# mfkiwl/GPS-JAMMING

Measured on AMD Instinct MI355X. Metric: Msamples/s uint8 I/Q through PSD+TDOA xcorr, higher is better.
Workload: dtype f32

## Files before the change

### gps-jamming_amd/csrc/k_scan.hip

```cpp
#include <type_traits>

#include "gj_common.h"

namespace gj {

constexpr int kScanThreads = 256;
constexpr size_t kScanTile = 65536;

__device__ __forceinline__ void acc_moments(const uint4& q, unsigned& s2, unsigned& s1) {
    s2 = __builtin_amdgcn_udot4(q.x, q.x, s2, false);
    s2 = __builtin_amdgcn_udot4(q.y, q.y, s2, false);
    s2 = __builtin_amdgcn_udot4(q.z, q.z, s2, false);
    s2 = __builtin_amdgcn_udot4(q.w, q.w, s2, false);
    s1 = __builtin_amdgcn_udot4(q.x, 0x01010101u, s1, false);
    s1 = __builtin_amdgcn_udot4(q.y, 0x01010101u, s1, false);
    s1 = __builtin_amdgcn_udot4(q.z, 0x01010101u, s1, false);
    s1 = __builtin_amdgcn_udot4(q.w, 0x01010101u, s1, false);
}

__device__ __forceinline__ void block_byte_moments(const uint8_t* __restrict__ p, size_t begin, size_t end,
                                                   unsigned long long& s2_out, unsigned long long& s1_out) {
    __shared__ unsigned long long red[2][kScanThreads / 64];
    const int tid = threadIdx.x;
    unsigned s2 = 0, s1 = 0;
// ... 163 lines not shown
                    run_len = 0;
                }
                ++run_len;
            }
        });
        if (run_len) atomicAdd(&sh.hist[run_digit], run_len);
        __syncthreads();
        const unsigned h = sh.hist[tid];
        unsigned inc = h;
#pragma unroll
        for (int off = 1; off < 64; off <<= 1) {
            const unsigned o = __shfl_up(inc, off, 64);
            if ((tid & 63) >= off) inc += o;
        }
        if ((tid & 63) == 63) sh.wave_tot[tid >> 6] = inc;
        __syncthreads();
        unsigned base = 0;
        for (int w = 0; w < (tid >> 6); ++w) base += sh.wave_tot[w];
        const unsigned excl = base + inc - h;
        if (h && excl <= want && want < excl + h) { sh.digit = tid; sh.rest = want - excl; }
        __syncthreads();
        prefix |= sh.digit << shift;
        mask |= 255u << shift;
        want = sh.rest;
        __syncthreads();
    }
    return prefix;
}

__device__ __forceinline__ void power_threshold_body(const float* __restrict__ power, size_t n, float pct, float ratio,
                                                     float* __restrict__ stats, uint8_t* __restrict__ mask, ThrShared& sh) {
    const int tid = threadIdx.x;
    const bool cached = n <= (size_t)kThrCache;
    if (tid == 0) { sh.nan_flag = 0; sh.above = 0; sh.count_le = 0; sh.next_key = 0xffffffffu; }
    __syncthreads();
    unsigned reg[kThrPerThread];
    unsigned has_nan = 0;
    if (cached) {
#pragma unroll
        for (int j = 0; j < kThrPerThread; ++j) {
            const size_t i = (size_t)tid + (size_t)kThrThreads * j;
            const float p = (i < n) ? power[i] : 0.0f;
            has_nan |= (p != p);
            reg[j] = float_key(p);
        }
    } else {
#pragma unroll
        for (int j = 0; j < kThrPerThread; ++j) reg[j] = 0;
        for (size_t i = tid; i < n; i += kThrThreads) {
            const float p = power[i];
            has_nan |= (p != p);
        }
    }
    if (has_nan) atomicOr(&sh.nan_flag, 1u);
    const float q = pct / 100.0f;
    const float vidx = (float)(n - 1) * q;
    size_t lo = (size_t)floorf(vidx);
    if (lo > n - 1) lo = n - 1;
    const size_t hi = (lo + 1 < n) ? lo + 1 : n - 1;
    const float g = vidx - (float)lo;
    const unsigned ka = block_select(reg, power, cached, n, lo, sh);
    unsigned kb = ka;
    if (hi != lo) {
        unsigned cnt = 0, nxt = 0xffffffffu;
        thr_for_each(reg, power, cached, n, [&](unsigned k, size_t) {
            cnt += (k <= ka);
            if (k > ka && k < nxt) nxt = k;
        });
        cnt = wave_sum_u32(cnt);
#pragma unroll
        for (int off = 32; off > 0; off >>= 1) {
            const unsigned o = __shfl_xor(nxt, off, 64);
            nxt = o < nxt ? o : nxt;
        }
        if ((tid & 63) == 0) { atomicAdd(&sh.count_le, cnt); atomicMin(&sh.next_key, nxt); }
        __syncthreads();
        kb = (sh.count_le >= lo + 2) ? ka : sh.next_key;
    }
    if (tid == 0) {
        const float a = key_float(ka), b = key_float(kb);
        const float d = b - a;
        float base = (g >= 0.5f) ? (b - d * (1.0f - g)) : (a + d * g);
        if (sh.nan_flag) base = __builtin_nanf("");
        if (base <= 0.0f) base = 1.0f;
        const float thr = base * ratio;
        stats[0] = base;
        stats[1] = thr;
        sh.thr = thr;
    }
    __syncthreads();
    const float thr = sh.thr;
    unsigned cnt = 0;
    thr_for_each(reg, power, cached, n, [&](unsigned k, size_t i) {
        const bool hot = key_float(k) > thr;
        cnt += hot;
        if (mask) mask[i] = hot;
    });
    cnt = wave_sum_u32(cnt);
    if ((tid & 63) == 0) atomicAdd(&sh.above, (unsigned long long)cnt);
    __syncthreads();
    if (tid == 0) stats[2] = (float)sh.above;
}

__global__ __launch_bounds__(kThrThreads) __attribute__((amdgpu_num_vgpr(104))) void power_threshold_kernel(const float* __restrict__ power, size_t n, float pct,
                                                                      float ratio, float* __restrict__ stats,
                                                                      uint8_t* __restrict__ mask) {
    __shared__ ThrShared sh;
    power_threshold_body(power, n, pct, ratio, stats, mask, sh);
}

int launch_power_threshold(gj_ctx* ctx, const float* d_power, size_t n, float pct, float rise_db, float* d_stats,
                           uint8_t* d_mask) {
    if (n == 0) return fail(ctx, GJ_ERR_INVALID, "empty power map");
    const float ratio = (float)pow(10.0, (double)rise_db / 10.0);
    hipLaunchKernelGGL(power_threshold_kernel, dim3(1), dim3(kThrThreads), 0, ctx->stream, d_power, n, pct, ratio, d_stats,
                       d_mask);
    GJ_LAUNCH_CHECK(ctx);
    return GJ_OK;
}

__device__ __forceinline__ float amp_of(unsigned i8, unsigned q8, Unpack up) {
    const int vi = 2 * (int)i8 - up.off2, vq = 2 * (int)q8 - up.off2;
    return __fsqrt_rn((float)(vi * vi + vq * vq)) * up.half_scale;
}
__device__ __forceinline__ unsigned pk_minus_off2(int o2) { return ((unsigned)(-o2) & 0xffffu) * 0x10001u; }

template <int HI>
__device__ __forceinline__ float amp_of_half(unsigned w, unsigned k2, unsigned km255, float hs) {
    const unsigned spread = __builtin_amdgcn_perm(w, w, HI ? 0x0C030C02u : 0x0C010C00u);
    unsigned h;
    int m;
    asm("v_pk_mad_i16 %0, %1, %2, %3" : "=v"(h) : "v"(spread), "v"(k2), "v"(km255));
    asm("v_dot2_i32_i16 %0, %1, %1, 0" : "=v"(m) : "v"(h));
    return __fsqrt_rn((float)m) * hs;
}

__device__ __forceinline__ unsigned m_of(unsigned i8, unsigned q8, int o2 = 255) {
    const int vi = 2 * (int)i8 - o2, vq = 2 * (int)q8 - o2;
    return (unsigned)(vi * vi + vq * vq);
}

template <int HI>
__device__ __forceinline__ int msq_of_half(unsigned w, unsigned k2, unsigned km255) {
    const unsigned spread = __builtin_amdgcn_perm(w, w, HI ? 0x0C030C02u : 0x0C010C00u);
    unsigned h;
    int m;
    asm("v_pk_mad_i16 %0, %1, %2, %3" : "=v"(h) : "v"(spread), "v"(k2), "v"(km255));
    asm("v_dot2_i32_i16 %0, %1, %1, 0" : "=v"(m) : "v"(h));
    return m;
}

constexpr size_t kAmpTileSamples = kScanTile / 2;

struct AmpTile {
    double sum;
    long long first;
};

__device__ double block_sum_f64(double v, double* sh ) {
    v = wave_sum_f64(v);
    __syncthreads();
    if ((threadIdx.x & 63) == 0) sh[threadIdx.x >> 6] = v;
    __syncthreads();
    double t = 0.0;
    for (unsigned k = 0; k < blockDim.x / 64; ++k) t += sh[k];
    return t;
}

__device__ long long amp_block_first(const AmpTile* __restrict__ tiles, size_t ntiles, long long* first_s) {
    if (threadIdx.x == 0) *first_s = 0x7fffffffffffffffll;
    __syncthreads();
    long long f = 0x7fffffffffffffffll;
    for (size_t t = threadIdx.x; t < ntiles; t += 16 * (size_t)blockDim.x) {
        long long v[16];
#pragma unroll
        for (int k = 0; k < 16; ++k) {
            const size_t tt = t + (size_t)k * blockDim.x;
            v[k] = tt < ntiles ? tiles[tt].first : 0x7fffffffffffffffll;
        }
#pragma unroll
        for (int k = 0; k < 16; ++k) f = v[k] < f ? v[k] : f;
    }
    if (f != 0x7fffffffffffffffll) atomicMin(first_s, f);
    __syncthreads();
    return *first_s;
}

__device__ double amp_block_tail(const uint8_t* __restrict__ iq, size_t nsamples, const AmpTile* __restrict__ tiles,
                                 long long first, Unpack up, double* sh) {
    const size_t t0 = (size_t)first / kAmpTileSamples;
    if ((size_t)first == t0 * kAmpTileSamples) return tiles[t0].sum;
    const size_t e0 = ((t0 + 1) * kAmpTileSamples < nsamples) ? (t0 + 1) * kAmpTileSamples : nsamples;
    double acc = 0.0;
    for (size_t s = (size_t)first + threadIdx.x; s < e0; s += blockDim.x) acc += (double)amp_of(iq[2 * s], iq[2 * s + 1], up);
    return block_sum_f64(acc, sh);
}

__device__ double amp_block_total(const AmpTile* __restrict__ tiles, size_t ntiles, size_t t0, double* sh) {
    double acc = 0.0;
    for (size_t t = t0 + 1 + threadIdx.x; t < ntiles; t += 16 * (size_t)blockDim.x) {
        double v[16];
#pragma unroll
        for (int k = 0; k < 16; ++k) {
            const size_t tt = t + (size_t)k * blockDim.x;
            v[k] = tt < ntiles ? tiles[tt].sum : 0.0;
        }
#pragma unroll
        for (int g = 0; g < 2; ++g) {
            if (t + (size_t)(8 * g) * blockDim.x < ntiles)
                acc += ((v[8 * g] + v[8 * g + 1]) + (v[8 * g + 2] + v[8 * g + 3])) + ((v[8 * g + 4] + v[8 * g + 5]) + (v[8 * g + 6] + v[8 * g + 7]));
        }
    }
    return block_sum_f64(acc, sh);
}

static inline bool power_edge_value(size_t nchunks, size_t nbytes, size_t chunk_bytes, int flags, float* val) {
    if (!nchunks) return false;
    const size_t len = nbytes - (nchunks - 1) * chunk_bytes;
    if ((flags & GJ_CP_ODD_CHUNK_ZERO) && (len & 1)) { *val = 0.0f; return true; }
    if ((len >> 1) == 0) { *val = __builtin_nanf(""); return true; }
    return false;
}
__device__ __forceinline__ void amp_combine_body(const AmpTile* __restrict__ tiles, size_t ntiles,
                                                 const gj_amp_part* __restrict__ parts, int n_parts, size_t nsamples,
                                                 gj_amp_stats* __restrict__ out, double* sh) {
    long long first = 0x7fffffffffffffffll;
    double tail = 0.0;
    for (int p = 0; p < n_parts; ++p)
        if (parts[p].first_index >= 0 && parts[p].first_index < first) { first = parts[p].first_index; tail = parts[p].tail; }
    if (first == 0x7fffffffffffffffll) {
        if (threadIdx.x == 0) {
            out->first_index = -1; out->count = 0; out->sum = 0.0; out->mean = 0.f; out->reserved = 0.f;
        }
        return;
    }
    const double behind = amp_block_total(tiles, ntiles, (size_t)first / kAmpTileSamples, sh);
    if (threadIdx.x == 0) {
        const double total = behind + tail;
        const unsigned long long cnt = nsamples - (size_t)first;
        out->first_index = first;
        out->count = cnt;
        out->sum = total;
        out->mean = (float)(total / (double)cnt);
        out->reserved = 0.f;
    }
}

__global__ __launch_bounds__(256) void amp_combine_kernel(const AmpTile* __restrict__ tiles, size_t ntiles,
                                                           const gj_amp_part* __restrict__ parts, int n_parts,
                                                           size_t nsamples, gj_amp_stats* __restrict__ out) {
    __shared__ double sh[16];
    amp_combine_body(tiles, ntiles, parts, n_parts, nsamples, out, sh);
}

__global__ __launch_bounds__(kThrThreads) __attribute__((amdgpu_num_vgpr(104))) void combine_stats_kernel(
    const gj_combine_capture* __restrict__ caps, int n_captures, float pct, float ratio) {
    __shared__ ThrShared sh_thr;
    __shared__ double sh_amp[16];
    const int b = blockIdx.x;
    if (b < n_captures) {
        const gj_combine_capture c = caps[b];
        power_threshold_body(c.d_power, (size_t)c.n_chunks, pct, ratio, c.d_stats, nullptr, sh_thr);
    } else {
        const gj_combine_capture c = caps[b - n_captures];
        amp_combine_body(static_cast<const AmpTile*>(c.d_tiles), (size_t)c.n_tiles, c.d_amp_parts, c.n_parts,
                         (size_t)(c.total_bytes / 2), c.d_amp, sh_amp);
        if (threadIdx.x == 0) onset_combine(c.d_onset_parts, c.n_parts, c.d_onset);
    }
}

int launch_combine_stats(gj_ctx* ctx, const gj_combine_capture* d_caps, int n_captures, float pct, float rise_db) {
    const float ratio = (float)pow(10.0, (double)rise_db / 10.0);
    hipLaunchKernelGGL(combine_stats_kernel, dim3(2u * (unsigned)n_captures), dim3(kThrThreads), 0, ctx->stream, d_caps,
                       n_captures, pct, ratio);
    GJ_LAUNCH_CHECK(ctx);
    return GJ_OK;
}

constexpr int kOnsetOut = 2048;
constexpr int kOnsetMaxWin = 8192;

struct OnsetScratch {
    unsigned long long noise_S;
    float noise;
    float thr;
};

constexpr double kOnsetGuard = 1e-6;

__device__ __forceinline__ int onset_pad(int k) { return k + (k >> 5); }

typedef short gj_short2 __attribute__((ext_vector_type(2)));

__device__ __forceinline__ int wave_sum_lane63(int v) {
    v += __builtin_amdgcn_update_dpp(0, v, 0xB1, 0xf, 0xf, false);
    v += __builtin_amdgcn_update_dpp(0, v, 0x4E, 0xf, 0xf, false);
    v += __builtin_amdgcn_update_dpp(0, v, 0x141, 0xf, 0xf, false);
    v += __builtin_amdgcn_update_dpp(0, v, 0x140, 0xf, 0xf, false);
    v += __builtin_amdgcn_update_dpp(0, v, 0x142, 0xa, 0xf, false);
    v += __builtin_amdgcn_update_dpp(0, v, 0x143, 0xc, 0xf, false);
    return v;
}


template <bool TRACK_FIRST>
__global__ __launch_bounds__(kScanThreads) void stream_scan_kernel(const uint8_t* __restrict__ iq, size_t nsamples,
                                                                   size_t nbytes, size_t chunk_bytes,
                                                                   unsigned tiles_per_chunk, float eps, int flags,
                                                                   float* __restrict__ power,
                                                                   unsigned long long* __restrict__ acc, float thr,
                                                                   AmpTile* __restrict__ tiles,
                                                                   unsigned* __restrict__ cblk, Unpack up,
                                                                   unsigned skip_tiles, unsigned tile_base,
                                                                   unsigned noise_block, const uint8_t* __restrict__ noise_src,
                                                                   int noise_samples, OnsetScratch* __restrict__ sc) {
    if (blockIdx.x == noise_block) {
        unsigned long long s2 = 0, s1 = 0;
        block_byte_moments(noise_src, 0, (size_t)2 * noise_samples, s2, s1);
        if (threadIdx.x == 0)
            sc->noise_S = (unsigned long long)(4ll * (long long)s2 - 4ll * up.off2 * (long long)s1 + (long long)up.off2 * up.off2 * (2ll * noise_samples));
        return;
    }
    __shared__ unsigned long long red_m[2][kScanThreads / 64];
    __shared__ double red_s[kScanThreads / 64];
    __shared__ long long red_f[kScanThreads / 64];
    const int tid = threadIdx.x;
    const size_t t = (size_t)blockIdx.x + tile_base;
    const size_t b0 = t * kScanTile;
    const size_t use_end = 2 * nsamples;
    const size_t b1 = (b0 + kScanTile < use_end) ? b0 + kScanTile : use_end;
    const size_t nvec = (b1 - b0) >> 4;
    const uint4* v = reinterpret_cast<const uint4*>(iq + b0);
    unsigned S = 0;
    double sum = 0.0;
    long long first = 0x7fffffffffffffffll;
    unsigned k2 = 0x00020002u, km255 = pk_minus_off2(up.off2);
    asm volatile("" : "+v"(k2), "+v"(km255));
    auto body = [&](const uint4& q, unsigned i, const bool live) {
        const unsigned ws[4] = {q.x, q.y, q.z, q.w};
        int m[8];
#pragma unroll
        for (int k = 0; k < 4; ++k) {
            m[2 * k] = msq_of_half<0>(ws[k], k2, km255);
            m[2 * k + 1] = msq_of_half<1>(ws[k], k2, km255);
        }
        float part = 0.f;
#pragma unroll
        for (int k = 0; k < 8; ++k) {
            const float r = __fsqrt_rn((float)m[k]);
            part += r;
            if constexpr (TRACK_FIRST) {
                const long long idx = (long long)((b0 >> 1) + (size_t)i * 8 + k);
                if (live && r * up.half_scale > thr && idx < first) first = idx;
            }
        }
        const unsigned m8 = live ? (unsigned)(((m[0] + m[1]) + (m[2] + m[3])) + ((m[4] + m[5]) + (m[6] + m[7]))) : 0u;
        S += m8;
        const int c512 = wave_sum_lane63((int)m8);
        if ((tid & 63) == 63) cblk[(b0 >> 10) + (i >> 6)] = (unsigned)c512;
        sum += (double)(live ? part : 0.f);
    };
    if (nvec == kScanTile / 16) {
        for (unsigned i = tid; i < (unsigned)(kScanTile / 16); i += 4 * kScanThreads) {
            const uint4 q0 = v[i], q1 = v[i + kScanThreads], q2 = v[i + 2 * kScanThreads], q3 = v[i + 3 * kScanThreads];
            body(q0, i, true);
            body(q1, i + kScanThreads, true);
            body(q2, i + 2 * kScanThreads, true);
            body(q3, i + 3 * kScanThreads, true);
        }
    } else {
        const unsigned lane = tid & 63;
        for (unsigned ib = (unsigned)tid - lane; ib < (unsigned)nvec; ib += kScanThreads) {
            const unsigned i = ib + lane;
            const bool live = i < (unsigned)nvec;
            const uint4 q = live ? v[i] : uint4{0u, 0u, 0u, 0u};
            body(q, i, live);
        }
    }
    if (tid == 0 && (b0 + (nvec << 4)) < b1) {
        unsigned c = 0;
        for (size_t n = (b0 >> 1) + nvec * 8; 2 * n < b1; ++n) {
            const unsigned ui = iq[2 * n], uq = iq[2 * n + 1];
            const unsigned mm = m_of(ui, uq, up.off2);
            S += mm;
            c += mm;
            const float r = __fsqrt_rn((float)mm);
            sum += (double)r;
            if (TRACK_FIRST && r * up.half_scale > thr && (long long)n < first) first = (long long)n;
        }
        (void)c;
    }
    if (b1 == use_end && (b1 & 1023) != 0) {
        __syncthreads();
        if (tid < 64) {
            const size_t jb = (b1 - 1) >> 10;
            int c = 0;
            for (size_t n = jb * 512 + tid; n < nsamples; n += 64) c += (int)m_of(iq[2 * n], iq[2 * n + 1], up.off2);
            c = group_sum_dpp<64>(c);
            if (tid == 0) cblk[jb] = (unsigned)c;
        }
    }
    if constexpr (!TRACK_FIRST) {
        if (tid == 0 && b1 > b0) first = (long long)(b0 >> 1);
    }
    const unsigned long long mS = wave_sum_u64(S);
    sum = wave_sum_f64(sum);
#pragma unroll
    for (int off = 32; off > 0; off >>= 1) {
        const long long o = __shfl_xor(first, off, 64);
        first = o < first ? o : first;
    }
    if ((tid & 63) == 0) { red_m[0][tid >> 6] = mS; red_s[tid >> 6] = sum; red_f[tid >> 6] = first; }
    __syncthreads();
    if (tid == 0 && t >= skip_tiles) {
        const unsigned long long tS = red_m[0][0] + red_m[0][1] + red_m[0][2] + red_m[0][3];
        AmpTile at;
        at.sum = ((red_s[0] + red_s[1]) + (red_s[2] + red_s[3])) * (double)up.half_scale;
        long long f = red_f[0];
        for (int k = 1; k < 4; ++k) f = red_f[k] < f ? red_f[k] : f;
        at.first = (f == 0x7fffffffffffffffll) ? f : f - (long long)((size_t)skip_tiles * (kScanTile / 2));
        const size_t to = t - skip_tiles;
        tiles[to] = at;
        const size_t c = to / tiles_per_chunk;
        const size_t off = c * chunk_bytes;
        const size_t len = (nbytes - off < chunk_bytes) ? nbytes - off : chunk_bytes;
        const bool zero_rule = (flags & GJ_CP_ODD_CHUNK_ZERO) && ((len & 1) || len == 0);
        if (tiles_per_chunk == 1) {
            power[c] = zero_rule ? 0.0f : ((len >> 1) ? power_from_msum(tS, len >> 1, eps) : __builtin_nanf(""));
        } else {
            atomicAdd(&acc[2 * c], tS);
        }
    }
}

constexpr size_t kTailSlotBytes = 256u << 10;
constexpr size_t kTailPrioBytes = 256u << 20;
constexpr int kTailBlocks = 2048;
constexpr int kTailHalo = (kOnsetMaxWin + 510) / 512 + 1;
constexpr int kTailPre = kTailBlocks + kTailHalo + (kTailBlocks + kTailHalo) / 32 + 8;

struct TailRec {
    unsigned long long first;
    unsigned long long guard;
    unsigned below;
    unsigned pad;
};

struct TailArgs {
    const uint8_t* iq;
    unsigned long long nsamples;
    long long sample0;
    unsigned long long total_samples;
    unsigned long long slot_nsamples;
    int has_thr, is_part, valid, has_slot, hi_prio;
    float* power;
    unsigned long long nchunks;
    float pct, ratio;
    float* stats;
    uint8_t* mask;
    const uint8_t* own_iq;
    unsigned long long own_samples, own_tiles;
    const AmpTile* tiles;
    gj_amp_stats* amp;
    gj_amp_part* amp_part;
    long long own_sample0;
    int window, noise_samples, noise_in_scratch;
    float factor;
    const unsigned* cblk;
    OnsetScratch* sc;
    TailRec* rec;
    unsigned* arrive;
    unsigned nct;
    gj_onset* onset;
    uint8_t* slot;
    unsigned long long slice_samples;
    Unpack up;
};

struct TailShared {
    unsigned long long r64[2][kScanThreads / 64];
    unsigned r32[kScanThreads / 64];
    unsigned long long b64[2];
    unsigned b32;
    int last;
    long long start;
};

__device__ __forceinline__ unsigned long long block_min_u64(unsigned long long v, TailShared& sh, int slot) {
#pragma unroll
    for (int off = 32; off > 0; off >>= 1) {
        const unsigned long long o = __shfl_xor(v, off, 64);
        v = o < v ? o : v;
    }
    if ((threadIdx.x & 63) == 0) sh.r64[slot][threadIdx.x >> 6] = v;
    __syncthreads();
    unsigned long long r = sh.r64[slot][0];
#pragma unroll
    for (int k = 1; k < kScanThreads / 64; ++k) r = sh.r64[slot][k] < r ? sh.r64[slot][k] : r;
    __syncthreads();
    return r;
}
__device__ __forceinline__ unsigned block_max_u32(unsigned v, TailShared& sh) {
#pragma unroll
    for (int off = 32; off > 0; off >>= 1) {
        const unsigned o = __shfl_xor(v, off, 64);
        v = o > v ? o : v;
    }
    if ((threadIdx.x & 63) == 0) sh.r32[threadIdx.x >> 6] = v;
    __syncthreads();
    unsigned r = sh.r32[0];
#pragma unroll
    for (int k = 1; k < kScanThreads / 64; ++k) r = sh.r32[k] > r ? sh.r32[k] : r;
    __syncthreads();
    return r;
}
__device__ __forceinline__ unsigned long long block_sum_u64(unsigned long long v, TailShared& sh) {
    v = wave_sum_u64(v);
    if ((threadIdx.x & 63) == 0) sh.r64[0][threadIdx.x >> 6] = v;
    __syncthreads();
    unsigned long long r = 0;
#pragma unroll
    for (int k = 0; k < kScanThreads / 64; ++k) r += sh.r64[0][k];
    __syncthreads();
    return r;
}

__device__ __forceinline__ void block_min2_max(unsigned long long& a, unsigned long long& b, unsigned& c, TailShared& sh) {
#pragma unroll
    for (int off = 32; off > 0; off >>= 1) {
        const unsigned long long oa = __shfl_xor(a, off, 64), ob = __shfl_xor(b, off, 64);
        const unsigned oc = __shfl_xor(c, off, 64);
        a = oa < a ? oa : a;
        b = ob < b ? ob : b;
        c = oc > c ? oc : c;
    }
    if ((threadIdx.x & 63) == 0) { sh.r64[0][threadIdx.x >> 6] = a; sh.r64[1][threadIdx.x >> 6] = b; sh.r32[threadIdx.x >> 6] = c; }
    __syncthreads();
    a = sh.r64[0][0]; b = sh.r64[1][0]; c = sh.r32[0];
#pragma unroll
    for (int k = 1; k < kScanThreads / 64; ++k) {
        a = sh.r64[0][k] < a ? sh.r64[0][k] : a;
        b = sh.r64[1][k] < b ? sh.r64[1][k] : b;
        c = sh.r32[k] > c ? sh.r32[k] : c;
    }
    __syncthreads();
}

__device__ __forceinline__ void block_prefix_u32(unsigned* pre, unsigned* thread_tot, int need) {
    const int tid = threadIdx.x;
    const int per = (need + kScanThreads - 1) / kScanThreads;
    const int lo = tid * per;
    const int hi = (lo + per < need) ? lo + per : need;
    unsigned run = 0;
    for (int k = lo; k < hi; ++k) {
        run += pre[onset_pad(k + 1)];
        pre[onset_pad(k + 1)] = run;
    }
    thread_tot[tid] = run;
    __syncthreads();
    if (tid < 64) {
        unsigned t0 = thread_tot[4 * tid], t1 = thread_tot[4 * tid + 1], t2 = thread_tot[4 * tid + 2], t3 = thread_tot[4 * tid + 3];
        unsigned tot = t0 + t1 + t2 + t3, inc = tot;
#pragma unroll
        for (int off = 1; off < 64; off <<= 1) {
            const unsigned o = __shfl_up(inc, off, 64);
            if (tid >= off) inc += o;
        }
        const unsigned ex = inc - tot;
        thread_tot[4 * tid] = ex;
        thread_tot[4 * tid + 1] = ex + t0;
        thread_tot[4 * tid + 2] = ex + t0 + t1;
        thread_tot[4 * tid + 3] = ex + t0 + t1 + t2;
    }
    __syncthreads();
    const unsigned add = thread_tot[tid];
    for (int k = lo; k < hi; ++k) pre[onset_pad(k + 1)] += add;
    __syncthreads();
}

__device__ void tail_onset_range(const TailArgs& A, unsigned w, unsigned* pre_c, unsigned* thread_tot, unsigned* pre_x,
                                 TailShared& sh) {
    const int tid = threadIdx.x;
    const int window = A.window;
    const size_t nsamples = (size_t)A.nsamples;
    const size_t nout = nsamples - (size_t)window + 1;
    unsigned long long noise_S;
    if (A.noise_in_scratch) {
        noise_S = A.sc->noise_S;
    } else {
        const size_t nb = (size_t)A.noise_samples / 512;
        unsigned long long part = 0;
        for (size_t j = tid; j < nb; j += kScanThreads) part += A.cblk[j];
        for (size_t n = nb * 512 + tid; n < (size_t)A.noise_samples; n += kScanThreads) part += m_of(A.iq[2 * n], A.iq[2 * n + 1], A.up.off2);
        noise_S = block_sum_u64(part, sh);
    }
    float noise = (float)((double)noise_S / (4.0 * (double)A.noise_samples));
    if (noise == 0.f) noise = 1e-9f;
    const float thr_f = noise * A.factor;
    if (w == 0 && tid == 0) { A.sc->noise = noise; A.sc->thr = thr_f; }
    const double thr = (double)thr_f, thr_lo = thr * (1.0 - kOnsetGuard);
    const double scale = 0.25 / (double)window;
    const size_t j0 = (size_t)w * kTailBlocks;
    const int cb = (window + 510) / 512 + 1;
    const size_t nblk_total = (nsamples + 511) / 512;
    size_t jend = j0 + kTailBlocks;
    if (512 * jend > nout) jend = (nout + 511) / 512;
    const int nloc = jend > j0 ? (int)(jend - j0) : 0;
    const int need = nloc ? nloc + cb - 1 : 0;
    for (int k = tid; k < need; k += kScanThreads) {
        const size_t j = j0 + k;
        pre_c[onset_pad(k + 1)] = j < nblk_total ? A.cblk[j] : 0u;
    }
    if (tid == 0) pre_c[0] = 0;
    __syncthreads();
    if (need) block_prefix_u32(pre_c, thread_tot, need);
    unsigned long long first = ~0ull, guard = ~0ull;
    unsigned below = 0;
    const uint16_t* iq16_all = reinterpret_cast<const uint16_t*>(A.iq);
    int kstart = 0;
    while (kstart < nloc) {
        unsigned long long mine = ~0ull;
        for (int k = kstart + tid; k < nloc; k += kScanThreads) {
            const unsigned U = pre_c[onset_pad(k + cb)] - pre_c[onset_pad(k)];
            if ((double)U * scale > thr_lo) { mine = (unsigned long long)k; break; }
        }
        const unsigned long long k1u = block_min_u64(mine, sh, 0);
        const int k1 = k1u == ~0ull ? nloc : (int)k1u;
        unsigned quiet = 0;
        for (int k = kstart + tid; k < k1; k += kScanThreads) {
            const unsigned U = pre_c[onset_pad(k + cb)] - pre_c[onset_pad(k)];
            quiet = U > quiet ? U : quiet;
        }
        quiet = block_max_u32(quiet, sh);
        below = quiet > below ? quiet : below;
        if (k1 >= nloc) break;
        const size_t o0 = (j0 + (size_t)k1) * 512;
        size_t o1 = o0 + kOnsetOut;
        if (o1 > jend * 512) o1 = jend * 512;
        if (o1 > nout) o1 = nout;
        const int npos = (int)(o1 - o0);
        const int needx = npos + window - 1;
        const uint16_t* iq16 = iq16_all + o0;
        for (int k = tid; k < needx; k += kScanThreads) {
            const unsigned v = iq16[k];
            pre_x[onset_pad(k + 1)] = m_of(v & 255u, v >> 8, A.up.off2);
        }
        if (tid == 0) pre_x[0] = 0;
        __syncthreads();
        block_prefix_u32(pre_x, thread_tot, needx);
        unsigned Sv[kOnsetOut / kScanThreads];
        unsigned long long best = ~0ull, best_lo = ~0ull;
#pragma unroll
        for (int i = 0; i < kOnsetOut / kScanThreads; ++i) {
            const int k = tid + i * kScanThreads;
            Sv[i] = 0;
            if (k < npos) {
                const unsigned S = pre_x[onset_pad(k + window)] - pre_x[onset_pad(k)];
                Sv[i] = S;
                const double ma = (double)S * scale;
                if (ma > thr_lo && best_lo == ~0ull) best_lo = o0 + k;
                if (ma > thr && best == ~0ull) best = o0 + k;
            }
        }
        unsigned long long hit = best, hit_lo = best_lo;
        unsigned b = 0;
#pragma unroll
        for (int i = 0; i < kOnsetOut / kScanThreads; ++i) {
            const int k = tid + i * kScanThreads;
            if (k < npos && o0 + k < best) b = Sv[i] > b ? Sv[i] : b;
        }
        block_min2_max(hit, hit_lo, b, sh);
        if (hit != ~0ull) {
            b = 0;
#pragma unroll
            for (int i = 0; i < kOnsetOut / kScanThreads; ++i) {
                const int k = tid + i * kScanThreads;
                if (k < npos && o0 + k < hit) b = Sv[i] > b ? Sv[i] : b;
            }
            b = block_max_u32(b, sh);
        }
        below = b > below ? b : below;
        if (hit_lo != ~0ull && guard == ~0ull) guard = hit_lo;
        if (hit != ~0ull) { first = hit; break; }
        kstart = k1 + (npos + 511) / 512;
    }
    if (tid == 0) {
        TailRec r;
        r.first = first; r.guard = guard; r.below = below; r.pad = 0;
        A.rec[w] = r;
    }
}

__device__ void tail_onset_finish(const TailArgs& A, TailShared& sh) {
    const int tid = threadIdx.x;
    const int window = A.window;
    if (A.valid) {
        unsigned long long wmin = ~0ull;
        for (unsigned w = tid; w < A.nct; w += kScanThreads)
            if (A.rec[w].first != ~0ull) { wmin = w; break; }
        const unsigned long long wstar = block_min_u64(wmin, sh, 0);
        const bool found = wstar != ~0ull;
        const unsigned wlast = found ? (unsigned)wstar : A.nct - 1;
        unsigned below = 0;
        unsigned long long guard = ~0ull;
        for (unsigned w = tid; w <= wlast; w += kScanThreads) {
            const TailRec r = A.rec[w];
            below = r.below > below ? r.below : below;
            guard = r.guard < guard ? r.guard : guard;
        }
        below = block_max_u32(below, sh);
        guard = block_min_u64(guard, sh, 1);
        const unsigned long long i0 = found ? A.rec[wstar].first : 0ull;
        unsigned long long S = 0;
        if (found)
            for (int k = tid; k < window; k += kScanThreads) S += m_of(A.iq[2 * (i0 + k)], A.iq[2 * (i0 + k) + 1], A.up.off2);
        S = block_sum_u64(S, sh);
        if (tid == 0) {
            const double thr = (double)A.sc->thr, scale = 0.25 / (double)window;
            gj_onset o;
            o.start_index = found ? A.sample0 + (long long)i0 + window / 2 : -1;
            o.noise_power = A.sc->noise;
            o.threshold = A.sc->thr;
// ... 420 lines not shown
```

Before: 406,000.

## Replace per-sample float threshold test with integer max and first-vector rescan

```diff
diff --git a/gps-jamming_amd/csrc/k_scan.hip b/gps-jamming_amd/csrc/k_scan.hip
--- a/gps-jamming_amd/csrc/k_scan.hip
+++ b/gps-jamming_amd/csrc/k_scan.hip
@@ -489,6 +489,18 @@
     return v;
 }
 
+__device__ __forceinline__ int first_hit_m(float half_scale, float thr) {
+    const int lane = (int)(threadIdx.x & 63);
+    int base = 0;
+#pragma unroll
+    for (int s = 1 << 18; s >= 1; s >>= 6) {
+        const bool hit = __fsqrt_rn((float)(base + lane * s)) * half_scale > thr;
+        const unsigned long long b = __ballot(hit);
+        const int j = b ? __ffsll((long long)b) - 1 : 64;
+        if (j) base += (j - 1) * s + 1;
+    }
+    return base;
+}
 
 template <bool TRACK_FIRST>
 __global__ __launch_bounds__(kScanThreads) void stream_scan_kernel(const uint8_t* __restrict__ iq, size_t nsamples,
@@ -510,8 +522,10 @@
     }
     __shared__ unsigned long long red_m[2][kScanThreads / 64];
     __shared__ double red_s[kScanThreads / 64];
-    __shared__ long long red_f[kScanThreads / 64];
+    __shared__ unsigned red_f[kScanThreads / 64];
     const int tid = threadIdx.x;
+    int m_hit = 0;
+    if constexpr (TRACK_FIRST) m_hit = first_hit_m(up.half_scale, thr);
     const size_t t = (size_t)blockIdx.x + tile_base;
     const size_t b0 = t * kScanTile;
     const size_t use_end = 2 * nsamples;
@@ -520,10 +534,12 @@
     const uint4* v = reinterpret_cast<const uint4*>(iq + b0);
     unsigned S = 0;
     double sum = 0.0;
+    constexpr unsigned kNoVec = 1u << 16;
+    unsigned firstv = kNoVec;
     long long first = 0x7fffffffffffffffll;
     unsigned k2 = 0x00020002u, km255 = pk_minus_off2(up.off2);
     asm volatile("" : "+v"(k2), "+v"(km255));
-    auto body = [&](const uint4& q, unsigned i, const bool live) {
+    auto body = [&](const uint4& q, const bool live, int& c512) -> int {
         const unsigned ws[4] = {q.x, q.y, q.z, q.w};
         int m[8];
 #pragma unroll
@@ -533,35 +549,46 @@
         }
         float part = 0.f;
 #pragma unroll
-        for (int k = 0; k < 8; ++k) {
-            const float r = __fsqrt_rn((float)m[k]);
-            part += r;
-            if constexpr (TRACK_FIRST) {
-                const long long idx = (long long)((b0 >> 1) + (size_t)i * 8 + k);
-                if (live && r * up.half_scale > thr && idx < first) first = idx;
-            }
-        }
+        for (int k = 0; k < 8; ++k) part += __fsqrt_rn((float)m[k]);
         const unsigned m8 = live ? (unsigned)(((m[0] + m[1]) + (m[2] + m[3])) + ((m[4] + m[5]) + (m[6] + m[7]))) : 0u;
         S += m8;
-        const int c512 = wave_sum_lane63((int)m8);
-        if ((tid & 63) == 63) cblk[(b0 >> 10) + (i >> 6)] = (unsigned)c512;
+        c512 = wave_sum_lane63((int)m8);
         sum += (double)(live ? part : 0.f);
+        int mx = 0;
+        if constexpr (TRACK_FIRST) mx = max(max(max(max(max(max(max(m[0], m[1]), m[2]), m[3]), m[4]), m[5]), m[6]), m[7]);
+        return mx;
     };
+    unsigned* const cb = cblk + (b0 >> 10) + (tid >> 6);
     if (nvec == kScanTile / 16) {
-        for (unsigned i = tid; i < (unsigned)(kScanTile / 16); i += 4 * kScanThreads) {
-            const uint4 q0 = v[i], q1 = v[i + kScanThreads], q2 = v[i + 2 * kScanThreads], q3 = v[i + 3 * kScanThreads];
-            body(q0, i, true);
-            body(q1, i + kScanThreads, true);
-            body(q2, i + 2 * kScanThreads, true);
-            body(q3, i + 3 * kScanThreads, true);
+        for (unsigned trip = 0; trip < 4; ++trip) {
+            const uint4* const vt = v + trip * (4 * kScanThreads);
+            const uint4 q0 = vt[tid], q1 = vt[tid + kScanThreads], q2 = vt[tid + 2 * kScanThreads], q3 = vt[tid + 3 * kScanThreads];
+            int c0, c1, c2, c3;
+            const int mx0 = body(q0, true, c0), mx1 = body(q1, true, c1), mx2 = body(q2, true, c2), mx3 = body(q3, true, c3);
+            if constexpr (TRACK_FIRST) {
+                unsigned cand = kNoVec;
+                if (mx3 >= m_hit) cand = 3;
+                if (mx2 >= m_hit) cand = 2;
+                if (mx1 >= m_hit) cand = 1;
+                if (mx0 >= m_hit) cand = 0;
+                firstv = min(firstv, cand + 4 * trip);
+            }
+            if ((tid & 63) == 63) {
+                unsigned* const ct = cb + 16 * trip;
+                ct[0] = (unsigned)c0; ct[4] = (unsigned)c1; ct[8] = (unsigned)c2; ct[12] = (unsigned)c3;
+            }
         }
     } else {
         const unsigned lane = tid & 63;
-        for (unsigned ib = (unsigned)tid - lane; ib < (unsigned)nvec; ib += kScanThreads) {
+        unsigned k = 0;
+        for (unsigned ib = (unsigned)tid - lane; ib < (unsigned)nvec; ib += kScanThreads, ++k) {
             const unsigned i = ib + lane;
             const bool live = i < (unsigned)nvec;
             const uint4 q = live ? v[i] : uint4{0u, 0u, 0u, 0u};
-            body(q, i, live);
+            int c;
+            const int mx = body(q, live, c);
+            if (TRACK_FIRST && live && mx >= m_hit) firstv = min(firstv, k);
+            if (lane == 63) cb[4 * k] = (unsigned)c;
         }
     }
     if (tid == 0 && (b0 + (nvec << 4)) < b1) {
@@ -592,19 +619,32 @@
     }
     const unsigned long long mS = wave_sum_u64(S);
     sum = wave_sum_f64(sum);
-#pragma unroll
-    for (int off = 32; off > 0; off >>= 1) {
-        const long long o = __shfl_xor(first, off, 64);
-        first = o < first ? o : first;
-    }
-    if ((tid & 63) == 0) { red_m[0][tid >> 6] = mS; red_s[tid >> 6] = sum; red_f[tid >> 6] = first; }
+    if constexpr (TRACK_FIRST) {
+        firstv = firstv < kNoVec ? (unsigned)tid + kScanThreads * firstv : 0xffffffffu;
+#pragma unroll
+        for (int off = 32; off > 0; off >>= 1) firstv = min(firstv, (unsigned)__shfl_xor((int)firstv, off, 64));
+    }
+    if ((tid & 63) == 0) { red_m[0][tid >> 6] = mS; red_s[tid >> 6] = sum; red_f[tid >> 6] = firstv; }
     __syncthreads();
     if (tid == 0 && t >= skip_tiles) {
         const unsigned long long tS = red_m[0][0] + red_m[0][1] + red_m[0][2] + red_m[0][3];
         AmpTile at;
         at.sum = ((red_s[0] + red_s[1]) + (red_s[2] + red_s[3])) * (double)up.half_scale;
-        long long f = red_f[0];
-        for (int k = 1; k < 4; ++k) f = red_f[k] < f ? red_f[k] : f;
+        long long f = first;
+        if constexpr (TRACK_FIRST) {
+            const unsigned fv = min(min(red_f[0], red_f[1]), min(red_f[2], red_f[3]));
+            if (fv != 0xffffffffu) {
+                const uint4 q = v[fv];
+                const unsigned ws[4] = {q.x, q.y, q.z, q.w};
+                int k = 7;
+#pragma unroll
+                for (int kk = 6; kk >= 0; --kk) {
+                    const int m = (kk & 1) ? msq_of_half<1>(ws[kk >> 1], k2, km255) : msq_of_half<0>(ws[kk >> 1], k2, km255);
+                    if (m >= m_hit) k = kk;
+                }
+                f = (long long)((b0 >> 1) + (size_t)fv * 8 + (size_t)k);
+            }
+        }
         at.first = (f == 0x7fffffffffffffffll) ? f : f - (long long)((size_t)skip_tiles * (kScanTile / 2));
         const size_t to = t - skip_tiles;
         tiles[to] = at;
```

Measured after the change: 404,900. No clear change (-0.3%).
